# tsolomko/SWCompression

Measured on AMD Instinct MI355X. Metric: decompressed GiB/s, higher is better.
Workload: dtype u8; 1 GPU; 100000 x 64 KiB gzip members (BASELINE configs[1]; 4096 distinct, tiled at distinct addresses); codec=deflate, units_per_gpu=100000, unit_bytes=65536, compressed_bytes_per_gpu=2122936095, decompressed_bytes_per_gpu=6553600000, parallelism=1 x independent shards (weak scaling)

## Files before the change

swcompression_amd/csrc/inflate_sync.h:

```cpp
#ifndef SWC_INFLATE_SYNC_H
#define SWC_INFLATE_SYNC_H

#include "inflate_lane.h"
#include "simt.h"
#include "sync_round.h"

namespace swc {
namespace inflate {

#ifndef SWC_SYNC_LIT_BITS
#define SWC_SYNC_LIT_BITS 10
#endif
constexpr int kSyncLitBits = SWC_SYNC_LIT_BITS, kSyncDistBits = 8;
constexpr uint32_t kSyncChunk = SWC_SYNC_CHUNK;
constexpr uint32_t kSyncRound = 64u * kSyncChunk;
constexpr uint32_t kSyncStage = (kSyncRound + 32u + 15u) & ~15u;
constexpr uint32_t kPosFail = 0xFFFFFFFFu;
#ifndef SWC_SYNC_WALK_BACK
#define SWC_SYNC_WALK_BACK 128
#endif
#ifndef SWC_COPY_REC
#define SWC_COPY_REC 16
#define SWC_COPY_LIT 8
#endif
constexpr uint32_t kSyncWalkBack = SWC_SYNC_WALK_BACK;
static_assert(kSyncChunk % 4 == 0 && kSyncChunk >= 36, "sub-chunks are whole dwords");

#ifndef SWC_SYNC_NO_PAIRS
#define SWC_SYNC_NO_PAIRS 0
#endif
#ifndef SWC_SYNC_NO_FOLLOW
#define SWC_SYNC_NO_FOLLOW 0
#endif
#ifndef SWC_SYNC_FOLLOW_HELD
#define SWC_SYNC_FOLLOW_HELD 0
#endif
#define SWC_SYNC_FOLLOW (SWC_SYNC_NO_FOLLOW ? 0 : SWC_SYNC_FOLLOW_HELD ? 2 : 1)
constexpr uint32_t kEntLenBit = (uint32_t)kSyncLitBits + 2u;
constexpr uint32_t kEntNotLen = ((1u << (kSyncLitBits - kSyncDistBits)) - 1u) << (kSyncDistBits + 2), kEntLen = 1u << kEntLenBit, kEntLit = 1u << 13, kEntDist = 1u << 29, kEntStop = 1u << 30, kEntTog = 1u << 31;
static_assert(kSyncLitBits > kSyncDistBits && kEntLenBit <= 12u, "the entry keeps bits 10 .. 12 for the table switch");
constexpr uint32_t kEntBaseShift = 14, kEntPosMask = kEntTog | kEntStop | 31u;
constexpr uint32_t kLitMask4 = ((1u << kSyncLitBits) - 1u) << 2, kDistMask4 = ((1u << kSyncDistBits) - 1u) << 2;
static_assert(kEntLen == 4u << kSyncLitBits, "the length flag is the byte offset of the distance table");
static_assert(((((uint32_t)kSyncLitBits + 2u) << 10) & kEntLen) != 0u && (kEntLit & (kEntLen | kEntNotLen)) == 0u, "a link has the literal bit AND the length bit, a literal only the first (the follow-up literal tells them apart by that)");
static_assert((kLitMask4 & ~kEntNotLen) == kDistMask4, "the masks differ in the not-length bits");
constexpr uint32_t kInvLit = 2u | kEntNotLen | kEntStop, kInvDist = kInvLit | kEntTog;
constexpr uint32_t kEntShShift = 23, kEntPairBit = 28, kEntPair = SWC_SYNC_NO_PAIRS ? 0u : 1u << kEntPairBit, kEntPairLenShift = 16, kPairLenMax = 127;
SWC_HD uint32_t make_entry(uint32_t clen, uint32_t ext, uint32_t kind, uint32_t mant, uint32_t sh) {
    const uint32_t c = (clen + ext + 2u) | ((clen + 2u) << 5);
    const uint32_t v = SWC_SYNC_NO_PAIRS ? (mant << sh) << kEntBaseShift : (mant << kEntBaseShift) | (sh << kEntShShift);
    return kind == 1 ? c | kEntNotLen | kEntLit | v
         : kind == 2 ? c | kEntLen | kEntTog | v
         : kind == 3 ? c | kEntNotLen | kEntStop
                     : c | kEntNotLen | kEntDist | kEntTog | v;
}
SWC_HD uint32_t ent_bits(uint32_t e) { return (e & 31u) - 2u; }
SWC_HD uint32_t ent_code_bits(uint32_t e) { return ((e >> 5) & 31u) - 2u; }
SWC_HD bool ent_is_eob(uint32_t e) { return (e & kEntStop) != 0u && (e & 31u) > 2u; }
SWC_HD bool ent_is_link(uint32_t e) { return (e & kEntPosMask) == 0u; }
SWC_HD bool ent_is_pair(uint32_t e) { return (e & kEntPair) != 0u; }
SWC_HD uint32_t ent_pair_len(uint32_t e) { return bfe32(e, kEntPairLenShift, 7); }
SWC_HD uint32_t ent_base(uint32_t e) {
    if (SWC_SYNC_NO_PAIRS) return bfe32(e, kEntBaseShift, 15);
    return bfe32(e, kEntBaseShift, ent_is_pair(e) ? 2u : 9u) << bfe32(e, kEntShShift, 4);
}
SWC_HD uint32_t pair_entry(uint32_t e, uint32_t idx, const uint32_t* dlut) {
    if (SWC_SYNC_NO_PAIRS || ent_is_link(e) || (e & (kEntLen | kEntStop)) != kEntLen) return 0u;
    const uint32_t nl = ent_bits(e), cl = ent_code_bits(e);
    if (nl >= (uint32_t)kSyncLitBits) return 0u;
    const uint32_t r = (uint32_t)kSyncLitBits - nl;
    const uint32_t len = ent_base(e) + ((idx >> cl) & ((1u << (nl - cl)) - 1u));
    if (len > kPairLenMax) return 0u;
    const uint32_t de = dlut[(idx >> nl) & ((1u << kSyncDistBits) - 1u)];
    if (ent_is_link(de) || (de & (kEntDist | kEntStop)) != kEntDist) return 0u;
    const uint32_t d = ent_code_bits(de);
    if (d > r) return 0u;
    const uint32_t c2 = nl + d + 2u, n2 = c2 + (ent_bits(de) - d);
    return n2 | (c2 << 5) | kEntNotLen | kEntDist | kEntPair | (len << kEntPairLenShift) | (de & ((3u << kEntBaseShift) | (15u << kEntShShift)));
}

SWC_HD uint32_t entry_of_symbol(bool dist, uint32_t sym, uint32_t d) {
    if (!dist) {
        if (sym < 256) return make_entry(d, 0, 1, sym, 0);
        if (sym == 256) return make_entry(d, 0, 3, 0, 0);
        if (sym > 285) return kInvLit;
        const uint32_t s = sym - 257u;
        const uint32_t e = s < 8 || s == 28 ? 0u : (s >> 2) - 1u;
        const uint32_t base = s < 8 ? 3u + s : s == 28 ? 258u : 3u + ((4u + (s & 3u)) << e);
        return make_entry(d, e, 2, base, 0);
    }
    if (sym > 29) return kInvDist;
    const uint32_t e = sym < 4 ? 0u : (sym >> 1) - 1u;
    return make_entry(d, e, 0, sym < 4 ? sym : 2u + (sym & 1u), e);
}

constexpr int kAuxLim = 0, kAuxSlot = 16, kAuxStart = 32, kAuxCount = 48 , kAuxOver = 49, kAuxTable = 52;
constexpr int kAuxLit = 0, kAuxDist = kAuxTable, kAuxWords = 2 * kAuxTable;
constexpr uint32_t kSpillSyms = 512, kSpillSub = 1536, kSubLds = 184, kSubMax = (uint32_t)(lzr::kProvSpillBytes - kSpillSub) / 4u;
constexpr uint32_t kSymDist = 288;
static_assert(kAuxWords * 4 <= (int)kSpillSyms && kSpillSyms + 2 * (288 + 32) <= kSpillSub && kSubMax < 4096u, "spill layout");

struct SyncLds {
    alignas(16) uint8_t stage[kSyncStage];
    uint32_t lut[(1 << kSyncLitBits) + (1 << kSyncDistBits)];
    uint32_t sub[kSubLds];
};
#if SWC_SYNC_CHUNK == 68 && SWC_SYNC_LIT_BITS == 10
static_assert(sizeof(SyncLds) == 10240, "16 waves per CU: the wave's LDS must stay within 160 KB / 16");
#endif
constexpr uint32_t kHdrLens = 0;
constexpr uint32_t kHdrRun = 320;
constexpr uint32_t kHdrClLut = 512;
constexpr uint32_t kHdrSorted = 640;
constexpr uint32_t kHdrRank = 1280;
constexpr uint32_t kHdrIn = 1280;
constexpr uint32_t kHdrPt = 1280;
constexpr uint32_t kHdrTab = 3840;
static_assert(kHdrTab + 2 * 33 * 4 <= kSyncStage && kHdrPt + 2 * 1280 <= kHdrTab, "header scratch fits the stage");

enum { kSyncEob = 0, kSyncBail = 1, kSyncBailCap = 2 };
#if defined(SWC_HOST_EMULATION)
inline uint64_t g_sync_stats[8];
#define SWC_SYNC_STAT(i, n) (g_sync_stats[i] += (n))
inline uint64_t g_sync_iters = 0, g_sync_wave[4] = {0, 0, 0, 0}, g_sync_passmax = 0, g_sync_it0 = 0;
inline uint8_t g_sync_long[4096];
#define SWC_SYNC_ITER() (g_sync_iters++)
#define SWC_SYNC_LONG() (g_sync_long[(g_sync_iters - 1 - g_sync_it0) & 4095] = 1)
#define SWC_SYNC_LANE_BEGIN(first) if (first) { g_sync_passmax = 0; for (auto& h_ : g_sync_long) h_ = 0; } g_sync_it0 = g_sync_iters;
#define SWC_SYNC_LANE_END(last, k) { if (g_sync_iters - g_sync_it0 > g_sync_passmax) g_sync_passmax = g_sync_iters - g_sync_it0; if (last) { g_sync_wave[k] += g_sync_passmax; for (auto h_ : g_sync_long) g_sync_wave[3] += h_; } }
#else
#define SWC_SYNC_STAT(i, n) ((void)0)
#define SWC_SYNC_ITER() ((void)0)
#define SWC_SYNC_LONG() ((void)0)
#define SWC_SYNC_LANE_BEGIN(first)
#define SWC_SYNC_LANE_END(last, k)
#endif
enum { kFlagEob = 1u, kFlagFail = 2u, kFlagTrap = 4u, kFlagSlow = 8u };
#if defined(SWC_PROFILE) && defined(__HIP_DEVICE_COMPILE__)
struct SyncProf {
    uint64_t acc[16] = {0, 0, 0, 0, 0, 0, 0, 0, 0, 0, 0, 0, 0, 0, 0, 0};
    uint64_t tlast = 0;
};
#define SWC_SP(pp, k) { const uint64_t t_ = __builtin_readcyclecounter(); (pp).acc[k] += t_ - (pp).tlast; (pp).tlast = t_; }
#define SWC_SPC(pp, k, n) ((pp).acc[k] += (n))
#else
struct SyncProf {};
#define SWC_SP(pp, k)
#define SWC_SPC(pp, k, n)
#endif

struct SubTab {
    const SWC_AS_GLOBAL uint32_t* g;
};
struct Spill {
    SWC_AS_GLOBAL uint32_t* aux;
    SWC_AS_GLOBAL uint16_t* syms;
    SWC_AS_GLOBAL uint32_t* sub;
};

SWC_D uint32_t stage_bits(const SyncLds* sl, uint32_t p) {
    const uint32_t* w = (const uint32_t*)(sl->stage + ((p >> 3) & 0x1FFCu));
    return funnel32(w[1], w[0], p);
}
SWC_D uint32_t long_lookup(const SyncLds* sl, const SubTab st, uint32_t bits4, uint32_t link) {
    const uint32_t idx = bfe32(bits4, link >> 10, link >> 5);
    const uint32_t at = (link >> 18) + idx;
    return st.g ? st.g[at] : sl->sub[at < kSubLds ? at : 0u];
}
SWC_D uint32_t entry_at(const SyncLds* sl, const SubTab st, uint32_t pos, bool dist, uint32_t& bits4) {
    bits4 = stage_bits(sl, pos);
    uint32_t e = *(const uint32_t*)((const uint8_t*)sl->lut + ((bits4 & (dist ? kDistMask4 : kLitMask4)) | (dist ? kEntLen : 0u)));
    if (ent_is_link(e)) e = long_lookup(sl, st, bits4, e);
    return e;
}

template <bool LIT>
SWC_D int decode_sym_canon(BitReader& br, const Spill sp) {
    const SWC_AS_GLOBAL uint32_t* tb = sp.aux + (LIT ? kAuxLit : kAuxDist);
    const uint32_t c15 = brev32(br.peek32()) >> 17;
    uint32_t len = 16, idx = 0;
    if (tb[kAuxOver] == 0) {
        len = 1;
#pragma unroll 1
        for (int d = 1; d <= 15; d++) len += c15 >= tb[kAuxLim + d] ? 1u : 0u;
        if (len > 15) return -1;
        idx = (tb[kAuxSlot + len] + (c15 >> (15 - len))) & 0xFFFFu;
    } else {
#pragma unroll 1
        for (uint32_t d = 1; d <= 15; d++) {
            const uint32_t st = tb[kAuxStart + d], cnt = (tb[kAuxStart + d + 1] - st) & 0xFFFFu;
            const uint32_t fst = d == 1 ? 0u : tb[kAuxLim + d - 1] >> (15 - d);
            const uint32_t k0 = ((c15 >> (15 - d)) - fst) & ((1u << d) - 1u);
            if (k0 < cnt) {
                len = d;
                idx = st + k0 + (((cnt - 1u - k0) >> d) << d);
                break;
            }
        }
        if (len > 15) return -1;
    }
    if (len > br.bc) return -1;
    br.consume(len);
    if (idx >= (LIT ? 288u : 32u)) return -1;
    return (int)sp.syms[(LIT ? 0u : kSymDist) + idx];
}

SWC_D int careful_step(Lane& ln, const Spill sp) {
    BitReader& br = ln.br;
    br.refill();
    const int sym = decode_sym_canon<true>(br, sp);
    if (sym < 0) return SWC_E_DEFLATE_SYMBOL_NOT_FOUND;
    if (sym < 256) {
        ln.put_byte((uint8_t)sym);
        return SWC_OK;
    }
    if (sym == 256) return -1;
    if (sym > 285) return SWC_E_DEFLATE_WRONG_SYMBOL;
    const uint32_t s = (uint32_t)sym - 257u;
    uint32_t length;
    if (s < 8) {
        length = 3 + s;
    } else if (s == 28) {
        length = 258;
    } else {
        const uint32_t e = (s >> 2) - 1;
        if (br.bc < e) return SWC_E_DEFLATE_SYMBOL_NOT_FOUND;
        length = 3 + ((4 + (s & 3)) << e) + br.bits(e);
    }
    br.refill();
    const int dc = decode_sym_canon<false>(br, sp);
    if (dc < 0) return SWC_E_DEFLATE_SYMBOL_NOT_FOUND;
    if (dc > 29) return SWC_E_DEFLATE_WRONG_SYMBOL;
    uint32_t distance;
    if (dc < 4) {
        distance = 1 + (uint32_t)dc;
    } else {
        const uint32_t e = ((uint32_t)dc >> 1) - 1;
        if (br.bc < e) return SWC_E_DEFLATE_SYMBOL_NOT_FOUND;
        distance = 1 + ((2 + ((uint32_t)dc & 1)) << e) + br.bits(e);
    }
    if ((uint64_t)distance > ln.pos) {
        const uint32_t over = distance - (uint32_t)ln.pos;
        if (over > ln.back) return SWC_E_REF_TRAP;
        if (over > ln.reach) ln.reach = over;
    }
    ln.emit_match(length, distance);
    return SWC_OK;
}

SWC_D void table_from_counts(const uint32_t* cnt, SWC_AS_GLOBAL uint32_t* tb, uint32_t* first, uint32_t* start) {
    uint32_t v = 0, off = 0, over = 0;
    tb[kAuxLim] = 0; tb[kAuxSlot] = 0; tb[kAuxStart] = 0;
    first[0] = 0; start[0] = 0;
#pragma unroll 1
    for (int d = 1; d <= 15; d++) {
        const uint32_t c = cnt[d];
        tb[kAuxLim + d] = (v + c) << (15 - d);
        if (c != 0 && v + c > (1u << d)) over = 1;
        tb[kAuxSlot + d] = (off - v) & 0xFFFFu;
        tb[kAuxStart + d] = off;
        first[d] = v;
        start[d] = off;
        off += c;
        v = (v + c) << 1;
    }
    tb[kAuxCount] = off;
    tb[kAuxOver] = over;
    start[16] = off;
}

SWC_D bool sync_tables_from_lengths(SyncLds* sl, const Spill sp, int literals, int distances, SubTab& st, SyncProf& pf) {
    SWC_SP(pf, 0)
    using simt::PT;
    constexpr int N = kWave;
    const uint8_t* lens = sl->stage + kHdrLens;
    uint32_t* run = (uint32_t*)(sl->stage + kHdrRun);
    uint16_t* sorted = (uint16_t*)(sl->stage + kHdrSorted);
    uint16_t* rankb = (uint16_t*)(sl->stage + kHdrRank);
    uint16_t* pt = (uint16_t*)(sl->stage + kHdrPt);
    uint32_t* tab = (uint32_t*)(sl->stage + kHdrTab);
    const int total = literals + distances;
    st.g = nullptr;
    SIMT_BEGIN(t, N) if (t < 32) run[t] = 0; SIMT_END_WAVE
    PT<uint32_t, N> v, upd;
    PT<uint64_t, N> m;
    PT<bool, N> p;
#pragma unroll 1
    for (int g = 0; g * N < literals + N; g++) {
        const bool is_dist = g * N >= literals;
        const int s0 = is_dist ? literals : g * N, s_end = is_dist ? total : literals;
        SIMT_BEGIN(t, N) v[t] = s0 + t < s_end ? (uint32_t)lens[s0 + t] : 0u; m[t] = ~0ull; SIMT_END
#pragma unroll
        for (int k = 0; k < 4; k++) {
            SIMT_BEGIN(t, N) p[t] = ((v[t] >> k) & 1u) != 0u; SIMT_END
            const uint64_t b = simt::wave_ballot<N>(p);
            SIMT_BEGIN(t, N) m[t] &= p[t] ? b : ~b; SIMT_END
        }
        SIMT_BEGIN(t, N)
            upd[t] = 0;
            if (v[t] != 0u) {
                const uint32_t rank = (uint32_t)simt::popc64(m[t] & ((1ull << t) - 1ull)), cnt = (uint32_t)simt::popc64(m[t]);
                const uint32_t base = run[(is_dist ? 16u : 0u) + v[t]];
                rankb[s0 + t] = (uint16_t)(base + rank);
                if (rank == cnt - 1u) upd[t] = base + cnt;
            }
        SIMT_END_WAVE
        SIMT_BEGIN(t, N) if (upd[t] != 0u) run[(is_dist ? 16u : 0u) + v[t]] = upd[t]; SIMT_END_WAVE
    }
    SWC_SP(pf, 10)
    SIMT_BEGIN(t, N)
        if (t < 2) table_from_counts(run + 16 * t, sp.aux + (t ? kAuxDist : kAuxLit), tab + 33 * t, tab + 33 * t + 16);
    SIMT_END_WAVE
    SIMT_BEGIN(t, N)
        for (int s = t; s < total; s += N) {
            const uint32_t d = lens[s];
            if (d) {
                const bool dd = s >= literals;
                const uint32_t j = (dd ? kSymDist : 0u) + tab[(dd ? 33 : 0) + 16 + d] + rankb[s];
                const uint32_t sym = (uint32_t)(s - (dd ? literals : 0));
                if (j < kSymDist + 32u) { sorted[j] = (uint16_t)(sym | (d << 9)); sp.syms[j] = (uint16_t)sym; }
            }
        }
        for (int i = t; i < (1 << kSyncLitBits) + (1 << kSyncDistBits); i += N) sl->lut[i] = i < (1 << kSyncLitBits) ? kInvLit : kInvDist;
    SIMT_END_WAVE
    simt::vmem_fence();
    SWC_SP(pf, 11)
    if (sp.aux[kAuxLit + kAuxOver] != 0u || sp.aux[kAuxDist + kAuxOver] != 0u) return false;
    uint32_t used = 0, used_lit = 0;
    PT<uint32_t, N> sz, rv, ln2;
#pragma unroll 1
    for (int tbl = 0; tbl < 2; tbl++) {
        const uint32_t root = tbl ? (uint32_t)kSyncDistBits : (uint32_t)kSyncLitBits, rmask = (1u << root) - 1u;
        const uint32_t* first = tab + 33 * tbl;
        const uint32_t* start = first + 16;
        const uint32_t n_sym = start[16] < (tbl ? 32u : 288u) ? start[16] : (tbl ? 32u : 288u);
        const uint16_t* srt = sorted + (tbl ? kSymDist : 0u);
        uint32_t* lut = sl->lut + (tbl ? (1 << kSyncLitBits) : 0);
        uint16_t* ptt = pt + (tbl ? (1 << kSyncLitBits) : 0);
#pragma unroll 1
        for (uint32_t j0 = 0; j0 < n_sym; j0 += (uint32_t)N) {
            SIMT_BEGIN(t, N)
                const uint32_t j = j0 + (uint32_t)t;
                sz[t] = 0; ln2[t] = 0; rv[t] = 0;
                if (j < n_sym) {
                    const uint32_t w = srt[j], sym = w & 511u, d = w >> 9;
                    const uint32_t code = first[d] + (j - start[d]);
                    const uint32_t rev = brev32(code) >> (32u - d);
                    rv[t] = rev; ln2[t] = d;
                    if (d <= root) {
                        const uint32_t entry = entry_of_symbol(tbl != 0, sym, d);
                        for (uint32_t q = rev; q <= rmask; q += 1u << d) lut[q] = entry;
                    } else {
                        bool last = j + 1u == n_sym;
                        if (!last) {
                            const uint32_t w2 = srt[j + 1u], d2 = w2 >> 9;
                            const uint32_t rev2 = brev32(first[d2] + (j + 1u - start[d2])) >> (32u - d2);
                            last = (rev2 & rmask) != (rev & rmask);
                        }
                        if (last) sz[t] = 1u << (d - root);
                    }
                }
            SIMT_END
            PT<uint32_t, N> x = sz;
            simt::wave_scan_incl<N>(x);
            SIMT_BEGIN(t, N)
                if (sz[t] != 0u) {
                    const uint32_t at = used + x[t] - sz[t], k = ln2[t] - root, pre = rv[t] & rmask;
                    if (at + sz[t] <= kSubMax) {
                        ptt[pre] = (uint16_t)(at | (k << 12));
                        lut[pre] = (k << 5) | ((root + 2u) << 10) | (at << 18);
                    }
                }
            SIMT_END
            used += simt::wave_read<N>(x, N - 1);
        }
        if (tbl == 0) used_lit = used;
    }
    SWC_SP(pf, 12)
    if (used > kSubMax) return false;
    SWC_AS_GLOBAL uint32_t* subg = used > kSubLds ? sp.sub : nullptr;
    st.g = subg;
    simt::wave_fence();
#if !SWC_SYNC_NO_PAIRS
    SIMT_BEGIN(t, N)
        for (int i = t; i < (1 << kSyncLitBits); i += N) {
            const uint32_t pe2 = pair_entry(sl->lut[i], (uint32_t)i, sl->lut + (1 << kSyncLitBits));
            if (pe2 != 0u) sl->lut[i] = pe2;
        }
    SIMT_END
#endif
    SIMT_BEGIN(t, N)
        for (uint32_t i = (uint32_t)t; i < used; i += (uint32_t)N) {
            const uint32_t inv = i < used_lit ? kInvLit : kInvDist;
            if (subg) subg[i] = inv; else sl->sub[i] = inv;
        }
    SIMT_END_WAVE
    if (subg) simt::vmem_fence();
#pragma unroll 1
    for (int tbl = 0; tbl < 2; tbl++) {
        const uint32_t root = tbl ? (uint32_t)kSyncDistBits : (uint32_t)kSyncLitBits, rmask = (1u << root) - 1u;
        const uint32_t* first = tab + 33 * tbl;
        const uint32_t* start = first + 16;
        const uint32_t n_sym = start[16] < (tbl ? 32u : 288u) ? start[16] : (tbl ? 32u : 288u);
        if (start[root + 1] >= n_sym) continue;
        const uint16_t* srt = sorted + (tbl ? kSymDist : 0u);
        const uint16_t* ptt = pt + (tbl ? (1 << kSyncLitBits) : 0);
        SIMT_BEGIN(t, N)
            for (uint32_t j = start[root + 1] + (uint32_t)t; j < n_sym; j += (uint32_t)N) {
                const uint32_t w = srt[j], sym = w & 511u, d = w >> 9;
                const uint32_t rev = brev32(first[d] + (j - start[d])) >> (32u - d);
                const uint32_t entry = entry_of_symbol(tbl != 0, sym, d);
                const uint32_t pw = ptt[rev & rmask], at = pw & 0xFFFu, k = pw >> 12;
                for (uint32_t q = rev >> root; q < (1u << k); q += 1u << (d - root)) {
                    if (subg) subg[at + q] = entry; else sl->sub[at + q] = entry;
                }
            }
        SIMT_END
    }
    simt::wave_fence();
    if (subg) simt::vmem_fence();
    SWC_SP(pf, 13)
    return true;
}

SWC_D uint32_t walk_chunk(const SyncLds* sl, const SubTab st, uint32_t start, uint32_t chunk_end, uint32_t in_bits) {
    if (chunk_end > in_bits) chunk_end = in_bits;
    if (start >= in_bits) return kPosFail;
    uint32_t pos = start, tm = kLitMask4, tb = 0, e = 0;
    uint32_t c_notlen = kEntNotLen, c_dmask = kDistMask4;
    SWC_OPAQUE(c_notlen); SWC_OPAQUE(c_dmask);
    if (start < chunk_end) do {
        SWC_SYNC_STAT(4, 1);
        SWC_SYNC_ITER();
        const uint32_t bits4 = stage_bits(sl, pos);
        e = *(const uint32_t*)((const uint8_t*)sl->lut + and_or(bits4, tm, tb));
        uint32_t mm = e & kEntPosMask;
        if (mm == 0u) { SWC_SYNC_STAT(7, 1); SWC_SYNC_LONG(); e = long_lookup(sl, st, bits4, e); mm = e & kEntPosMask; }
        pos = pos + mm + 0xFFFFFFFEu;
        tm = and_or(e, c_notlen, c_dmask);
        tb = e & kEntLen;
    } while ((int32_t)pos < (int32_t)chunk_end);
    const uint32_t endb = pos & 0x3FFFFFFFu;
    const bool fail = ((pos & kEntStop) != 0u && !ent_is_eob(e)) || endb > in_bits;
    return fail ? kPosFail : endb;
}

struct ProvOut {
    uint32_t end, nlit, nrec, nout, flags, tail;
    int32_t need;
};
using sround::kProvRow;

template <bool NEED>
SWC_D void decode_chunk_prov(const SyncLds* sl, const SubTab st, uint32_t start, uint32_t chunk_end, uint32_t in_bits, gptr prov,
                             uint32_t lane, uint32_t run0, ProvOut& r) {
    const uint32_t rbase = 4u * lane;
#if !SWC_SYNC_FOLLOW
    const uint32_t lbase = (uint32_t)lzr::kProvRecBytes + 4u * lane;
#endif
    uint32_t pos = start, tm = kLitMask4, tb = 0, e = 0;
#if SWC_SYNC_FOLLOW
    const uint32_t lbase4 = (uint32_t)lzr::kProvRecBytes - kProvRow + 4u * lane;
    uint32_t plen = 0, run = run0, nl4 = 4, nout = 0, lb = 0;
#else
    uint32_t plen = 0, run = run0, nl3 = 3, nout = 0, lb = 0;
#endif
    uint32_t roff = rbase + kProvRow;
    int32_t need = -0x40000000;
    uint32_t c_notlen = kEntNotLen, c_dmask = kDistMask4;
    int32_t c_m256 = -256;
    SWC_OPAQUE(c_notlen); SWC_OPAQUE(c_dmask); SWC_OPAQUE(c_m256);
#if !SWC_SYNC_NO_PAIRS
    int32_t c_m4 = -4;
    SWC_OPAQUE(c_m4);
#endif
    if (chunk_end > in_bits) chunk_end = in_bits;
    const bool dead = start >= in_bits;
    uint32_t w0 = 0, w1 = 0;
    if (!dead && start < chunk_end) { const uint32_t* w = (const uint32_t*)(sl->stage + ((pos >> 3) & 0x1FFCu)); w0 = w[0]; w1 = w[1]; }
    if (!dead && start < chunk_end) do {
        SWC_SYNC_STAT(5, 1);
        SWC_SYNC_ITER();
        const uint32_t bits4 = funnel32(w1, w0, pos);
        e = *(const uint32_t*)((const uint8_t*)sl->lut + and_or(bits4, tm, tb));
        uint32_t mm = e & kEntPosMask;
        if (mm == 0u) { SWC_SYNC_STAT(7, 1); SWC_SYNC_LONG(); e = long_lookup(sl, st, bits4, e); mm = e & kEntPosMask; }
#if SWC_SYNC_FOLLOW == 2
        const uint32_t wbase = pos & ~31u;
#endif
        pos = pos + mm + 0xFFFFFFFEu;
#if SWC_SYNC_FOLLOW == 2
        const uint32_t fb4 = (uint32_t)((((uint64_t)w1 << 32) | w0) >> ((pos - wbase) & 63u));
        const uint32_t fend = wbase + (65u - kEntLenBit) < chunk_end ? wbase + (65u - kEntLenBit) : chunk_end;
#else
        { const uint32_t* w = (const uint32_t*)(sl->stage + ((pos >> 3) & 0x1FFCu)); w0 = w[0]; w1 = w[1]; }
#endif
        tm = and_or(e, c_notlen, c_dmask);
        tb = e & kEntLen;
#if SWC_SYNC_FOLLOW
#if SWC_SYNC_FOLLOW != 2
        const uint32_t fb4 = funnel32(w1, w0, pos);
        const uint32_t fend = chunk_end;
#endif
        const uint32_t f = *(const uint32_t*)((const uint8_t*)sl->lut + (fb4 & kLitMask4));
        const uint32_t fm = ((uint32_t)(pos < fend) & (uint32_t)((f & (kEntLit | kEntLen)) == kEntLit)) != 0u ? f : 2u;
        pos = pos + (fm & 31u) + 0xFFFFFFFEu;
        { const uint32_t* w = (const uint32_t*)(sl->stage + ((pos >> 3) & 0x1FFCu)); w0 = w[0]; w1 = w[1]; }
#endif
#if SWC_SYNC_NO_PAIRS
        const uint32_t val = (bfe32(bits4, 0, e) >> ((e >> 5) & 31u)) + bfe32(e, kEntBaseShift, 15);
        const uint32_t mlen = plen;
#else
        const uint32_t lp = bfe32(e, kEntPairLenShift, 7) & sbfe1(e, kEntPairBit);
        const uint32_t val = lshl_add_v(mad24(lp, c_m4, bfe32(e, kEntBaseShift, 9)), bfe32(e, kEntShShift, 4), bfe32(bits4, 0, e) >> ((e >> 5) & 31u));
        const uint32_t mlen = plen + lp;
#endif
        const uint32_t lit1 = bfe32(e, 13, 1);
        lb = alignbyte32(val, lb, lit1);
        const uint32_t dm = sbfe1(e, 29);
#if SWC_SYNC_FOLLOW
        const uint32_t lit2 = bfe32(fm, 13, 1), byte2 = fm >> kEntBaseShift, nl4_0 = nl4, litn = lit1 + lit2;
        nl4 += litn;
        if ((nl4 ^ nl4_0) > 3u) store_u32(prov + lshl_add<6>(nl4 & ~3u, lbase4), alignbyte32(byte2, lb, clear_if(nl4, lit2)));
        lb = alignbyte32(byte2, lb, lit2);
#else
        nl3 += lit1;
        const uint32_t litn = lit1;
        if (((nl3 & 3u) | (lit1 << 2)) == 7u) store_u32(prov + lshl_add<6>(nl3 & ~3u, lbase), lb);
#endif
        if (dm != 0u) store_u32(prov + roff, lshl_add<7>(mlen, lshl_add<16>(val, run)));
        roff = mad24(dm, c_m256, roff);
        if (NEED) {
            const int32_t nd = (int32_t)val - (int32_t)nout;
            need = (int32_t)bfi32(dm, (uint32_t)(nd > need ? nd : need), (uint32_t)need);
        }
        nout += litn + mlen;
#if SWC_SYNC_FOLLOW
        run = bfi32(dm, lit2, run + litn);
#else
        run = clear_if(dm, run + lit1);
#endif
        plen = val & sbfe1(e, kEntLenBit);
    } while ((int32_t)pos < (int32_t)chunk_end);
#if SWC_SYNC_FOLLOW
    const uint32_t nlit = nl4 - 4u;
    if (nlit & 3u) store_u32(prov + lshl_add<6>((nl4 & ~3u) + 4u, lbase4), lb);
#else
    const uint32_t nlit = nl3 - 3u;
    if (nlit & 3u) store_u32(prov + lshl_add<6>(nl3 & ~3u, lbase), lb);
#endif
    const uint32_t endb = pos & 0x3FFFFFFFu;
    uint32_t flags = 0;
    if (dead) flags = kFlagFail;
    else if (pos & kEntStop) flags = ent_is_eob(e) ? kFlagEob : kFlagFail;
    uint32_t tail = 0;
    if (run > 0) {
        if (flags & kFlagEob) tail = run;
        else { store_u32(prov + roff, lzr::make_lits(run)); roff += kProvRow; }
    }
    if (endb > in_bits) flags |= kFlagFail;
    if (nlit + run0 > lzr::kLitRunMax) flags |= kFlagSlow;
    r.end = (flags & kFlagFail) ? kPosFail : endb;
    r.nlit = nlit; r.nrec = (roff - rbase) / kProvRow - 1u; r.nout = nout; r.flags = flags; r.tail = tail; r.need = need;
}

SWC_D void copy_prov(gcptr plit, gcptr prec, uint32_t nlit, uint32_t nrec, gptr ldst, SWC_AS_GLOBAL uint32_t* rdst) {
    sround::copy_prov<SWC_COPY_REC, SWC_COPY_LIT, true>(plit, prec, nlit, nrec, ldst, rdst);
}

struct ChunkOut {
    uint32_t end;
    uint32_t nlit, nrec, nout;
    uint32_t flags;
    uint32_t over;
};
template <int MODE, bool BIG, bool CHK>
SWC_D void decode_chunk(const SyncLds* sl, const SubTab st, uint32_t start, uint32_t chunk_end, uint32_t in_bits, gptr lit_dst,
                        SWC_AS_GLOBAL uint32_t* rec_dst, uint64_t out_pos0, ChunkOut& r, uint32_t back = 0) {
    uint32_t pos = start;
    bool dist_next = false;
    uint32_t plen = 0, run = 0, nlit = 0, nrec = 0, nout = 0, flags = 0, over = 0;
    uint32_t lb = 0, lbn = 0;
    const uint32_t own = out_pos0 > 0x40000000ull ? 0x40000000u : (uint32_t)out_pos0;
    const uint32_t room = own + back;
    for (;;) {
        if (!dist_next && pos >= chunk_end) break;
        SWC_SYNC_STAT(4 + MODE, 1);
        SWC_SYNC_ITER();
        uint32_t bits4;
        const uint32_t e = entry_at(sl, st, pos, dist_next, bits4);
        const uint32_t n = ent_bits(e);
        if ((e & kEntStop) || (CHK && pos + n > in_bits)) {
            if (!ent_is_eob(e) || (CHK && pos + n > in_bits)) flags |= kFlagFail;
            else { pos += n; flags |= kFlagEob; }
            break;
        }
        const bool was_dist = dist_next || ent_is_pair(e);
        if (ent_is_pair(e)) plen = ent_pair_len(e);
        const uint32_t is_lit = (e >> 13) & 1u;
        const uint32_t val = (bfe32(bits4, 0, e) >> ((e >> 5) & 31u)) + ent_base(e) + (was_dist ? 1u : 0u);
        if (MODE != 0 && was_dist && val > own + nout) {
            if (val > room + nout) { flags |= kFlagTrap; break; }
            if (val - (own + nout) > over) over = val - (own + nout);
        }
        const bool big = BIG && was_dist && run > lzr::kLitRunMax;
        if (MODE == 1) {
            if (is_lit) {
                lb = funnel32(val, lb, 8);
                if (++lbn == 4) { store_u32(lit_dst, lb); lit_dst += 4; lbn = 0; }
            }
            if (was_dist) {
                if (big) *rec_dst++ = lzr::make_lits(run);
                *rec_dst++ = lzr::make_match(big ? 0u : run, plen, val);
            }
        }
        nlit += is_lit;
        nout += is_lit + (was_dist ? plen : 0u);
        nrec += was_dist ? (big ? 2u : 1u) : 0u;
        run = was_dist ? 0u : run + is_lit;
        plen = (e & kEntLen) ? val : plen;
        dist_next = (e & kEntLen) != 0u;
        pos += n;
    }
    if (run > 0) {
        nrec++;
        if (MODE == 1) *rec_dst++ = lzr::make_lits(run);
    }
    if (MODE == 1) {
        for (uint32_t i = 0; i < lbn; i++) lit_dst[i] = (uint8_t)(lb >> (8 * (4u - lbn + i)));
    }
    r.end = (flags & kFlagFail) ? kPosFail : pos;
    r.nlit = nlit; r.nrec = nrec; r.nout = nout;
    r.flags = flags;
    r.over = over;
}

template <int N>
SWC_D void stage_round(SyncLds* sl, gcptr in, uint32_t in_len, uint32_t B, uint32_t first_start, simt::PT<uint32_t, N>& start) {
    using simt::PT;
    constexpr uint32_t kParts = (kSyncStage + 16u * N - 1u) / (16u * N);
    PT<uint64_t, N> sa[kParts], sb[kParts];
    PT<uint32_t, N> sp[kParts];
    SIMT_BEGIN(t, N)
#pragma unroll
        for (uint32_t k = 0; k < kParts; k++) {
            const uint32_t o = 16u * (uint32_t)t + k * 16u * N;
            uint64_t a = 0, b = 0;
            uint32_t prev = 0;
            const uint64_t at = (uint64_t)B + o;
            if (o < kSyncStage) {
                if (at + 16 <= in_len) {
                    a = load_u64(in + at); b = load_u64(in + at + 8);
                    if (o != 0) prev = load_u32(in + at - 4);
                } else {
                    for (uint32_t q = 0; q < 8; q++) if (at + q < in_len) a |= (uint64_t)in[at + q] << (8 * q);
                    for (uint32_t q = 0; q < 8; q++) if (at + 8 + q < in_len) b |= (uint64_t)in[at + 8 + q] << (8 * q);
                    if (o != 0) for (uint32_t q = 0; q < 4; q++) if (at - 4 + q < in_len) prev |= (uint32_t)in[at - 4 + q] << (8 * q);
                }
            }
            sa[k][t] = a; sb[k][t] = b; sp[k][t] = prev;
        }
    SIMT_END
    SIMT_BEGIN(t, N)
#pragma unroll
        for (uint32_t k = 0; k < kParts; k++) {
            const uint32_t o = 16u * (uint32_t)t + k * 16u * N;
            if (o < kSyncStage) {
                uint32_t* st32 = (uint32_t*)(sl->stage + o);
                const uint64_t a = sa[k][t], b = sb[k][t];
                const uint32_t w0 = (uint32_t)a, w1 = (uint32_t)(a >> 32), w2 = (uint32_t)b, w3 = (uint32_t)(b >> 32);
                st32[0] = funnel32(w0, sp[k][t], 30); st32[1] = funnel32(w1, w0, 30); st32[2] = funnel32(w2, w1, 30); st32[3] = funnel32(w3, w2, 30);
            }
        }
        start[t] = t == 0 ? first_start : (uint32_t)t * kSyncChunk * 8u - kSyncWalkBack;
    SIMT_END_WAVE
}
SWC_D bool redo_lane(int t, uint32_t& start, uint32_t pe, bool have) {
    const bool todo = t == 0 ? !have : pe != kPosFail && (start != pe || !have);
    if (todo && t != 0) start = pe;
    return todo;
}
SWC_D bool stopped_in_front(uint32_t start, uint32_t chunk_end) { return start + kSyncChunk * 8u < chunk_end; }
template <class R>
SWC_D void nothing_taken(R& r) {
    r = R{};
    r.end = kPosFail; r.flags = kFlagFail;
}
template <int N>
SWC_D bool prov_turn(int t, const SyncLds* sl, const SubTab st, uint32_t in_bits, gptr prov, bool need, uint32_t run0,
                     simt::PT<uint32_t, N>& start, const simt::PT<uint32_t, N>& pe, simt::PT<bool, N>& have, simt::PT<uint32_t, N>& endp,
                     simt::PT<uint32_t, N>& c_lit, simt::PT<uint32_t, N>& c_rec, simt::PT<uint32_t, N>& c_out, simt::PT<uint32_t, N>& flg,
                     simt::PT<uint32_t, N>& c_tail, simt::PT<uint32_t, N>& c_need) {
    if (!redo_lane(t, start[t], pe[t], have[t])) return false;
    ProvOut r;
    const uint32_t ce = ((uint32_t)t + 1u) * kSyncChunk * 8u;
    if (stopped_in_front(start[t], ce)) nothing_taken(r);
    else if (need) decode_chunk_prov<true>(sl, st, start[t], ce, in_bits, prov, (uint32_t)t, run0, r);
    else decode_chunk_prov<false>(sl, st, start[t], ce, in_bits, prov, (uint32_t)t, run0, r);
    endp[t] = r.end; c_lit[t] = r.nlit; c_rec[t] = r.nrec; c_out[t] = r.nout; flg[t] = r.flags;
    c_tail[t] = r.tail; c_need[t] = (uint32_t)r.need;
    have[t] = true;
    return true;
}

#ifndef SWC_TEAM_WAVES
#define SWC_TEAM_WAVES 6
#endif
#if defined(SWC_HOST_EMULATION)
inline uint64_t g_team_adopted = 0;
#define SWC_TEAM_STAT() (g_team_adopted++)
#else
#define SWC_TEAM_STAT() ((void)0)
#endif
constexpr int kTeamWaves = SWC_TEAM_WAVES;
constexpr uint32_t kTeamStride = 63u * kSyncChunk;
constexpr size_t kTeamProvBytes = lzr::kProvRecBytes + lzr::kProvLitBytes;
struct TeamRound {
    uint32_t c_lit[kWave], c_rec[kWave];
    uint32_t nv, eob, ok;
    uint32_t start1;
    uint32_t end_last, tail_last;
    uint32_t tot_lit, tot_rec, tot_out;
    uint32_t mneed;
// ... 330 lines not shown
                        else decode_chunk<0, true, false>(sl, st, start[t], ce, in_bits, nullptr, nullptr, 0, r);
                    }
                    endp[t] = r.end; c_lit[t] = r.nlit; c_rec[t] = r.nrec; c_out[t] = r.nout; flg[t] = r.flags;
                    have[t] = true;
                }
                SWC_SYNC_LANE_END(t_i_ == N - 1, 1)
            SIMT_END
            SWC_SP(pf, 3)
        }
        if (bail) { SWC_SYNC_STAT(1, 1); break; }
        SWC_SYNC_STAT(0, 1);
        const sround::Totals tot = sround::lane_offsets<N>(0u, nv, c_lit, c_rec, c_out, x_lit, x_rec, x_out);
        SWC_SP(pf, 4)
        const bool beyond = pos >= ln.cap;
        if (!beyond && pos + tot.out > ln.cap) { result = kSyncBailCap; break; }
        if (!beyond && (uint64_t)nrec + tot.rec > ln.max_rec) break;
        SIMT_BEGIN(t, N)
            SWC_SYNC_LANE_BEGIN(t_i_ == 0)
            if ((uint32_t)t < nv) {
                ChunkOut r;
                const uint32_t ce = ((uint32_t)t + 1u) * kSyncChunk * 8u;
                const uint64_t p0 = pos + (x_out[t] - c_out[t]);
                const bool bigs = c_lit[t] > lzr::kLitRunMax;
                if (beyond) decode_chunk<2, false, true>(sl, st, start[t], ce, in_bits, nullptr, nullptr, p0, r, back);
                else if (bigs || chk) decode_chunk<1, true, true>(sl, st, start[t], ce, in_bits, ln.lits + nlit + (x_lit[t] - c_lit[t]), ln.recs + nrec + (x_rec[t] - c_rec[t]), p0, r, back);
                else decode_chunk<1, false, false>(sl, st, start[t], ce, in_bits, ln.lits + nlit + (x_lit[t] - c_lit[t]), ln.recs + nrec + (x_rec[t] - c_rec[t]), p0, r, back);
                flg[t] = r.flags;
                c_need[t] = r.over;
            }
            SWC_SYNC_LANE_END(t_i_ == N - 1, 2)
        SIMT_END
        SWC_SP(pf, 5)
        SIMT_BEGIN(t, N) pb[t] = (uint32_t)t < nv && (flg[t] & kFlagTrap) != 0; SIMT_END
        if (simt::wave_ballot<N>(pb)) break;
        if (back != 0u && pos < 32768u) {
            SIMT_BEGIN(t, N) c_need[t] = (uint32_t)t < nv ? c_need[t] : 0u; SIMT_END
            simt::wave_scan_max_incl<N>(c_need);
            const uint32_t rr = simt::wave_read<N>(c_need, N - 1);
            if (rr > ln.reach) ln.reach = rr;
        }
        pos += tot.out;
        if (!beyond) { nlit += tot.lit; nrec += tot.rec; }
        P = 8ull * B + simt::wave_read<N>(endp, (int)nv - 1);
        ln.last_end = pos < ln.cap ? pos : (ln.last_end > ln.cap ? ln.last_end : ln.cap);
        if (eob) { result = kSyncEob; break; }
    }
    ln.pos = pos;
    ln.nlit = nlit;
    ln.nrec = nrec;
    ln.br.seek(P);
    return result;
}

SWC_D int build_dynamic_par(Lane& ln, SyncLds* sl, const Spill sp, SubTab& st, bool& fast, SyncProf& pf) {
    using simt::PT;
    constexpr int N = kWave;
    BitReader& br = ln.br;
    br.refill();
    if (br.bc < 14) return SWC_E_DEFLATE_SYMBOL_NOT_FOUND;
    const int literals = (int)br.bits(5) + 257;
    if (literals > 286) return SWC_E_DEFLATE_WRONG_SYMBOL;
    const int distances = (int)br.bits(5) + 1;
    const int ncl = (int)br.bits(4) + 4;
    br.refill();
    const uint64_t total_left = (uint64_t)br.len * 8 - br.consumed_bits();
    if (total_left < (uint64_t)(3 * ncl)) return SWC_E_DEFLATE_SYMBOL_NOT_FOUND;
    const uint8_t order[19] = {16, 17, 18, 0, 8, 7, 9, 6, 10, 5, 11, 4, 12, 3, 13, 2, 14, 1, 15};
    uint64_t clens = 0;
    for (int i = 0; i < ncl; i++) {
        br.refill();
        clens |= (uint64_t)br.bits(3) << (3 * order[i]);
    }
    Lane::ClTable cl;
    {
        uint64_t cnt8 = 0, runp = 0;
        for (int s = 0; s < 19; s++) {
            const uint32_t len = (uint32_t)(clens >> (3 * s)) & 7u;
            if (len) cnt8 += 1ull << (8 * len);
        }
        uint32_t v = 0, off = 0;
        cl.slot[0] = 0;
#pragma unroll
        for (int d = 1; d <= 7; d++) {
            const uint32_t c = (uint32_t)(cnt8 >> (8 * d)) & 255u;
            cl.slot[d] = ((v & 0x7FFFu) << 9) | off;
            runp |= (uint64_t)off << (8 * d);
            off += c;
            v = (v + c) << 1;
        }
        cl.slot[8] = off;
        cl.sym_lo = cl.sym_hi = 0;
        for (int s = 0; s < 19; s++) {
            const uint32_t len = (uint32_t)(clens >> (3 * s)) & 7u;
            if (len) {
                const uint32_t p = (uint32_t)(runp >> (8 * len)) & 255u;
                runp += 1ull << (8 * len);
                if (p < 12) cl.sym_lo |= (uint64_t)s << (5 * p);
                else cl.sym_hi |= (uint64_t)s << (5 * (p - 12));
            }
        }
    }
    SWC_SP(pf, 14)
    uint8_t* lens = sl->stage + kHdrLens;
    uint8_t* cl_lut = sl->stage + kHdrClLut;
    uint32_t* hin = (uint32_t*)(sl->stage + kHdrIn);
    const int total = literals + distances;
    const uint64_t end_bits = (uint64_t)br.len * 8;
    uint64_t W = simt::uniform(br.consumed_bits());
    gcptr in = br.in;
    const uint32_t in_len = br.len;
    SIMT_BEGIN(t, N)
        for (int i = t; i < 80; i += N) ((uint32_t*)lens)[i] = 0;
        for (int x = t; x < 128; x += N) {
            uint32_t len;
            const int idx = Lane::cl_lookup(cl, brev32((uint32_t)x) >> 17, len);
            const uint32_t sym = idx < 0 ? 0u : (uint32_t)((idx < 12 ? cl.sym_lo >> (5 * idx) : cl.sym_hi >> (5 * (idx - 12))) & 31u);
            cl_lut[x] = idx < 0 ? (uint8_t)0xFF : (uint8_t)(len | (sym << 3));
        }
    SIMT_END_WAVE
    SWC_SP(pf, 15)
    int n = 0;
    uint32_t prev = 0;
    uint64_t HB = ~0ull;
    PT<uint32_t, N> nxt, mlo, mhi, jmp, gl, gh, gj, src, symv, repv, errv, cbx, bef, key, kex;
    PT<bool, N> pb, actv;
    while (n < total) {
        if (HB == ~0ull || W + 64 + 32 > 8 * (HB + 1024)) {
            HB = (W >> 3) & ~3ull;
            SIMT_BEGIN(t, N)
                uint64_t a = 0, b = 0;
                const uint64_t at = HB + 16u * (uint32_t)t;
                if (at + 16 <= in_len) { a = load_u64(in + at); b = load_u64(in + at + 8); }
                else {
                    for (uint32_t k = 0; k < 8; k++) if (at + k < in_len) a |= (uint64_t)in[at + k] << (8 * k);
                    for (uint32_t k = 0; k < 8; k++) if (at + 8 + k < in_len) b |= (uint64_t)in[at + 8 + k] << (8 * k);
                }
                uint32_t* h4 = hin + 4 * t;
                h4[0] = (uint32_t)a; h4[1] = (uint32_t)(a >> 32); h4[2] = (uint32_t)b; h4[3] = (uint32_t)(b >> 32);
                if (t < 4) hin[256 + t] = 0;
            SIMT_END_WAVE
        }
        const uint32_t rel0 = (uint32_t)(W - 8 * HB);
        const uint64_t left64 = end_bits - W;
        const uint32_t left = left64 > 0xFFFFu ? 0xFFFFu : (uint32_t)left64;
        SIMT_BEGIN(t, N)
            const uint32_t rel = rel0 + (uint32_t)t;
            const uint32_t* w = hin + (rel >> 5);
            const uint32_t bits = funnel32(w[1], w[0], rel);
            const uint32_t e = cl_lut[bits & 127u];
            const uint32_t len = e & 7u, sym = e == 0xFFu ? 0u : e >> 3;
            const uint32_t xb = sym == 16u ? 2u : sym == 17u ? 3u : sym == 18u ? 7u : 0u;
            const uint32_t xv = bfe32(bits, len, xb);
            const uint32_t avail = left > (uint32_t)t ? left - (uint32_t)t : 0u;
            symv[t] = sym;
            repv[t] = sym < 16u ? 1u : sym == 18u ? 11u + xv : 3u + xv;
            errv[t] = e == 0xFFu || len > avail ? 1u : len + xb > avail ? 2u : 0u;
            nxt[t] = (uint32_t)t + (e == 0xFFu ? 1u : len + xb);
            jmp[t] = nxt[t];
            mlo[t] = t < 32 ? 1u << t : 0u;
            mhi[t] = t < 32 ? 0u : 1u << (t - 32);
        SIMT_END
#pragma unroll 1
        for (int k = 0; k < 6; k++) {
            if (simt::uniform(simt::wave_read<N>(jmp, 0)) >= 64u) break;
            SIMT_BEGIN(t, N) src[t] = jmp[t] < 64u ? jmp[t] : (uint32_t)t; SIMT_END
            simt::wave_gather<N>(gl, mlo, src);
            simt::wave_gather<N>(gh, mhi, src);
            simt::wave_gather<N>(gj, jmp, src);
            SIMT_BEGIN(t, N) if (jmp[t] < 64u) { mlo[t] |= gl[t]; mhi[t] |= gh[t]; jmp[t] = gj[t]; } SIMT_END
        }
        const uint64_t V = ((uint64_t)simt::uniform(simt::wave_read<N>(mhi, 0)) << 32) | simt::uniform(simt::wave_read<N>(mlo, 0));
        SIMT_BEGIN(t, N) cbx[t] = (V >> t) & 1ull ? repv[t] : 0u; SIMT_END
        simt::wave_scan_incl<N>(cbx);
        SIMT_BEGIN(t, N)
            const bool vis = ((V >> t) & 1ull) != 0ull;
            const uint32_t rep = repv[t], before = (uint32_t)n + cbx[t] - (vis ? rep : 0u), sym = symv[t];
            const bool act = vis && before < (uint32_t)total;
            uint32_t err = 0;
            if (act) {
                if (errv[t] == 1u) err = (uint32_t)SWC_E_DEFLATE_SYMBOL_NOT_FOUND;
                else if (sym == 16u && before == 0u) err = (uint32_t)SWC_E_DEFLATE_WRONG_SYMBOL;
                else if (sym >= 16u && errv[t] == 2u) err = (uint32_t)SWC_E_DEFLATE_SYMBOL_NOT_FOUND;
                else if (sym == 16u && before + rep > (uint32_t)total) err = (uint32_t)SWC_E_DEFLATE_WRONG_SYMBOL;
            }
            errv[t] = err;
            pb[t] = err != 0u;
            actv[t] = act;
            bef[t] = before;
            key[t] = act && sym != 16u ? (((uint32_t)t + 1u) << 8) | (sym < 16u ? sym : 0u) : 0u;
        SIMT_END
        {
            const uint64_t m_err = simt::wave_ballot<N>(pb);
            if (m_err) return (int)simt::wave_read<N>(errv, simt::ctz64(m_err));
        }
        kex = key;
        simt::wave_scan_max_incl<N>(kex);
        const uint32_t klast = simt::uniform(simt::wave_read<N>(kex, N - 1));
        simt::wave_shift_up<N>(key, kex, 0u);
        SIMT_BEGIN(t, N)
            if (actv[t]) {
                const uint32_t sym = symv[t];
                const uint32_t val = sym < 16u ? sym : sym == 16u ? (key[t] ? key[t] & 255u : prev) : 0u;
                if (val != 0u) for (uint32_t k = 0; k < repv[t]; k++) lens[bef[t] + k] = (uint8_t)val;
            }
        SIMT_END
        const uint64_t m_act = simt::wave_ballot<N>(actv);
        const int last = 63 - simt::clz64(m_act);
        n = (int)(simt::uniform(simt::wave_read<N>(bef, last)) + simt::uniform(simt::wave_read<N>(repv, last)));
        W += simt::uniform(simt::wave_read<N>(nxt, last));
        if (klast) prev = klast & 255u;
    }
    if (n != total) return SWC_E_DEFLATE_WRONG_SYMBOL;
    simt::wave_fence();
    br.seek(W);
    SWC_SP(pf, 0)
    fast = sync_tables_from_lengths(sl, sp, literals, distances, st, pf);
    return SWC_OK;
}

SWC_D void build_static_par(SyncLds* sl, const Spill sp, SubTab& st, bool& fast, SyncProf& pf) {
    constexpr int N = kWave;
    uint8_t* lens = sl->stage + kHdrLens;
    SIMT_BEGIN(t, N)
        for (int s = t; s < 320; s += N) lens[s] = (uint8_t)(s < 144 ? 8 : s < 256 ? 9 : s < 280 ? 7 : s < 288 ? 8 : 5);
    SIMT_END_WAVE
    fast = sync_tables_from_lengths(sl, sp, 288, 32, st, pf);
}

template <bool TEAM = false>
SWC_D void inflate_sync_job(Job& job, SyncLds* sl, uint8_t* ws, size_t ws_bytes, int lane, int lanes, uint64_t* prof = nullptr, Team* tm = nullptr) {
    Lane ln;
    SyncProf pf;
#if defined(SWC_PROFILE) && defined(__HIP_DEVICE_COMPILE__)
    pf.tlast = __builtin_readcyclecounter();
#endif
    ln.wlane = lane;
    ln.wlanes = lanes;
    ln.l = LaneLds{nullptr, 1};
    ln.out = (gptr)job.out;
    ln.cap = job.out_cap;
    ln.pos = 0;
    ln.nrec = 0;
    ln.nlit = 0;
    ln.last_end = 0;
    const size_t lo = ws ? lzr::lit_offset(ws_bytes, job.out_cap) : 0;
    ln.recs = (SWC_AS_GLOBAL uint32_t*)(ws + sizeof(lzr::StreamHeader));
    size_t rec_end = lo;
    ln.prov = nullptr;
    if (lo >= sizeof(lzr::StreamHeader) + 256 + lzr::kProvBytes) {
        rec_end = (lo - lzr::kProvBytes) & ~(size_t)15;
        ln.prov = (gptr)(ws + rec_end);
    }
    ln.max_rec = rec_end > sizeof(lzr::StreamHeader) ? (uint32_t)((rec_end - sizeof(lzr::StreamHeader)) / 4) : 0u;
    ln.lits = (gptr)(ws + lo);
    Spill sp{nullptr, nullptr, nullptr};
    if (ln.prov) {
        gptr s0 = ln.prov + lzr::kProvRecBytes + lzr::kProvLitBytes;
        sp.aux = (SWC_AS_GLOBAL uint32_t*)s0;
        sp.syms = (SWC_AS_GLOBAL uint16_t*)(s0 + kSpillSyms);
        sp.sub = (SWC_AS_GLOBAL uint32_t*)(s0 + kSpillSub);
    }
    int st = SWC_OK;
    const bool open = (job.aux & kDeflateOpen) != 0;
    bool ended_open = false;
    const bool linked = (job.aux & kDeflateLinked) != 0;
    ln.back = linked ? 32768u : 0u;
    if (linked && (job.aux & kDeflateJoined) == 0) {
        st = SWC_E_INVALID_ARGUMENT;
        ln.br.init((gcptr)job.in, 0, 0);
    } else if (lo == 0 || ln.prov == nullptr) {
        st = SWC_E_NEED_WORKSPACE;
        ln.br.init((gcptr)job.in, 0, 0);
    } else if (job.in_len > 0xFFFFFFF0ull) {
        st = SWC_E_INVALID_ARGUMENT;
        ln.br.init((gcptr)job.in, 0, 0);
    } else {
        ln.br.init((gcptr)job.in, (uint32_t)job.in_len, 0);
        if ((uint64_t)ln.br.len * 8 < 10) st = SWC_E_DEFLATE_WRONG_BLOCK_TYPE;
        while (st == SWC_OK) {
            ln.br.refill();
            if (open && ln.br.bc == 0) { ended_open = true; break; }
            if (ln.br.bc < 3) { st = SWC_E_REF_TRAP; break; }
            const uint32_t is_last = ln.br.bits(1);
            const uint32_t type = ln.br.bits(2);
            if (type == 0) {
                st = ln.run_stored();
            } else if (type == 1 || type == 2) {
                SWC_SP(pf, 6)
                bool fast = false;
                SubTab stb{nullptr};
                if (type == 1) build_static_par(sl, sp, stb, fast, pf);
                else st = build_dynamic_par(ln, sl, sp, stb, fast, pf);
                SWC_SP(pf, 1)
                if constexpr (TEAM) if (tm != nullptr) tm->gen++;
                if (st == SWC_OK) {
                    for (;;) {
                        if (fast) {
                            const int r = sync_block<TEAM>(ln, sl, stb, pf, tm);
                            if (r == kSyncEob) break;
                            if (r == kSyncBail) fast = false;
                        }
                        const uint64_t until = fast && ln.pos < ln.cap ? ln.cap : ~0ull;
                        int s2 = SWC_OK;
                        do { s2 = careful_step(ln, sp); } while (s2 == SWC_OK && ln.pos < until && until != ~0ull);
                        if (s2 == -1) break;
                        if (s2) { st = s2; break; }
                    }
                }
            } else {
                st = SWC_E_DEFLATE_WRONG_BLOCK_TYPE;
            }
            if (st != SWC_OK || is_last) break;
        }
        ln.flush_tail();
    }
    if constexpr (TEAM) if (tm != nullptr && tm->sh != nullptr) team_dismiss(*tm);
    if (ln.nrec > ln.max_rec) {
        st = SWC_E_NEED_WORKSPACE;
        ln.nrec = ln.max_rec;
    }
    if (st == SWC_OK && ln.pos > ln.cap) st = SWC_E_CAPACITY;
    if (ws && ws_bytes >= sizeof(lzr::StreamHeader) && (lane == 0)) {
        SWC_AS_GLOBAL lzr::StreamHeader* h = (SWC_AS_GLOBAL lzr::StreamHeader*)ws;
        h->nrec = ln.nrec;
        h->pad0 = ln.reach;
        h->nlit = ln.nlit;
    }
#if defined(SWC_PROFILE) && defined(__HIP_DEVICE_COMPILE__)
    SWC_SP(pf, 6)
    if (prof && lane == 0) for (int k = 0; k < 16; k++) prof[k] = pf.acc[k];
#else
    (void)prof; (void)pf;
#endif
    const uint64_t bits = ln.br.consumed_bits();
    const uint64_t consumed = (bits + 7) >> 3;
    job.in_consumed = consumed > job.in_len ? job.in_len : consumed;
    job.out_len = ln.pos;
    job.status = st;
    if (!ended_open) job.aux &= ~kDeflateOpen;
}

}
}
#endif
```

Before: 472.6 GiB/s.

## Parallelize Huffman count tables with wave scans and skip redundant LUT invalidation

Replaces the serial two-lane table_from_counts loop with wave-wide inclusive scans over the 32 length counts, computing limit, start and first codes per lane and detecting oversubscription with a ballot. The invalid-entry prefill of the lit/dist LUTs now runs only when the code is incomplete or over-subscribed, and overflowing subtable prefixes are invalidated directly. The pair-entry loop visits rows in bit-reversed order. The global memory fence moves from the table build to the end of the build and before the careful-step path. This is meant to cut per-block dynamic header cost, with some risk to correctness around fence placement and incomplete codes.

```diff
diff --git a/swcompression_amd/csrc/inflate_sync.h b/swcompression_amd/csrc/inflate_sync.h
--- a/swcompression_amd/csrc/inflate_sync.h
+++ b/swcompression_amd/csrc/inflate_sync.h
@@ -246,27 +246,6 @@
     }
     ln.emit_match(length, distance);
     return SWC_OK;
-}
-
-SWC_D void table_from_counts(const uint32_t* cnt, SWC_AS_GLOBAL uint32_t* tb, uint32_t* first, uint32_t* start) {
-    uint32_t v = 0, off = 0, over = 0;
-    tb[kAuxLim] = 0; tb[kAuxSlot] = 0; tb[kAuxStart] = 0;
-    first[0] = 0; start[0] = 0;
-#pragma unroll 1
-    for (int d = 1; d <= 15; d++) {
-        const uint32_t c = cnt[d];
-        tb[kAuxLim + d] = (v + c) << (15 - d);
-        if (c != 0 && v + c > (1u << d)) over = 1;
-        tb[kAuxSlot + d] = (off - v) & 0xFFFFu;
-        tb[kAuxStart + d] = off;
-        first[d] = v;
-        start[d] = off;
-        off += c;
-        v = (v + c) << 1;
-    }
-    tb[kAuxCount] = off;
-    tb[kAuxOver] = over;
-    start[16] = off;
 }
 
 SWC_D bool sync_tables_from_lengths(SyncLds* sl, const Spill sp, int literals, int distances, SubTab& st, SyncProf& pf) {
@@ -308,9 +287,40 @@
         SIMT_BEGIN(t, N) if (upd[t] != 0u) run[(is_dist ? 16u : 0u) + v[t]] = upd[t]; SIMT_END_WAVE
     }
     SWC_SP(pf, 10)
+    PT<uint32_t, N> cc, lim, off;
     SIMT_BEGIN(t, N)
-        if (t < 2) table_from_counts(run + 16 * t, sp.aux + (t ? kAuxDist : kAuxLit), tab + 33 * t, tab + 33 * t + 16);
+        cc[t] = t < 32 ? run[t] : 0u;
+        lim[t] = cc[t] << (15 - (t & 15));
+        off[t] = cc[t];
+    SIMT_END
+    simt::wave_scan_incl<N>(lim);
+    simt::wave_scan_incl<N>(off);
+    const uint32_t lim_lit = simt::uniform(simt::wave_read<N>(lim, 15)), off_lit = simt::uniform(simt::wave_read<N>(off, 15));
+    const uint32_t lim_dist = simt::uniform(simt::wave_read<N>(lim, 31)) - lim_lit;
+    SIMT_BEGIN(t, N)
+        if (t >= 16) { lim[t] -= lim_lit; off[t] -= off_lit; }
+        p[t] = t < 32 && cc[t] != 0u && lim[t] > (1u << 15);
+    SIMT_END
+    const uint32_t over_mask = (uint32_t)simt::wave_ballot<N>(p);
+    const bool over = over_mask != 0u;
+    SIMT_BEGIN(t, N)
+        if (t < 32) {
+            const uint32_t d = (uint32_t)t & 15u, a = (uint32_t)t >> 4;
+            const uint32_t first = (lim[t] - (cc[t] << (15u - d))) >> (15u - d), start = off[t] - cc[t];
+            SWC_AS_GLOBAL uint32_t* tb = sp.aux + (a ? kAuxDist : kAuxLit);
+            tb[kAuxLim + d] = lim[t];
+            tb[kAuxSlot + d] = (start - first) & 0xFFFFu;
+            tb[kAuxStart + d] = start;
+            tab[33u * a + d] = first;
+            tab[33u * a + 16u + d] = start;
+            if (d == 15u) {
+                tb[kAuxCount] = off[t];
+                tb[kAuxOver] = ((over_mask >> (16u * a)) & 0xFFFFu) != 0u ? 1u : 0u;
+                tab[33u * a + 32u] = off[t];
+            }
+        }
     SIMT_END_WAVE
+    const bool fill_lit = over || lim_lit != (1u << 15), fill_dist = over || lim_dist != (1u << 15);
     SIMT_BEGIN(t, N)
         for (int s = t; s < total; s += N) {
             const uint32_t d = lens[s];
@@ -321,11 +331,11 @@
                 if (j < kSymDist + 32u) { sorted[j] = (uint16_t)(sym | (d << 9)); sp.syms[j] = (uint16_t)sym; }
             }
         }
-        for (int i = t; i < (1 << kSyncLitBits) + (1 << kSyncDistBits); i += N) sl->lut[i] = i < (1 << kSyncLitBits) ? kInvLit : kInvDist;
+        if (fill_lit) for (int i = t; i < (1 << kSyncLitBits); i += N) sl->lut[i] = kInvLit;
+        if (fill_dist) for (int i = t; i < (1 << kSyncDistBits); i += N) sl->lut[(1 << kSyncLitBits) + i] = kInvDist;
     SIMT_END_WAVE
-    simt::vmem_fence();
     SWC_SP(pf, 11)
-    if (sp.aux[kAuxLit + kAuxOver] != 0u || sp.aux[kAuxDist + kAuxOver] != 0u) return false;
+    if (over) return false;
     uint32_t used = 0, used_lit = 0;
     PT<uint32_t, N> sz, rv, ln2;
 #pragma unroll 1
@@ -369,6 +379,8 @@
                     if (at + sz[t] <= kSubMax) {
                         ptt[pre] = (uint16_t)(at | (k << 12));
                         lut[pre] = (k << 5) | ((root + 2u) << 10) | (at << 18);
+                    } else {
+                        lut[pre] = tbl ? kInvDist : kInvLit;
                     }
                 }
             SIMT_END
@@ -383,14 +395,17 @@
     simt::wave_fence();
 #if !SWC_SYNC_NO_PAIRS
     SIMT_BEGIN(t, N)
-        for (int i = t; i < (1 << kSyncLitBits); i += N) {
-            const uint32_t pe2 = pair_entry(sl->lut[i], (uint32_t)i, sl->lut + (1 << kSyncLitBits));
+        for (int r = t; r < (1 << kSyncLitBits); r += N) {
+            const uint32_t i = brev32((uint32_t)r) >> (32u - (uint32_t)kSyncLitBits);
+            const uint32_t pe2 = pair_entry(sl->lut[i], i, sl->lut + (1 << kSyncLitBits));
             if (pe2 != 0u) sl->lut[i] = pe2;
         }
     SIMT_END
 #endif
     SIMT_BEGIN(t, N)
-        for (uint32_t i = (uint32_t)t; i < used; i += (uint32_t)N) {
+        uint32_t i0 = (uint32_t)t;
+        SWC_OPAQUE(i0);
+        for (uint32_t i = i0; i < used; i += (uint32_t)N) {
             const uint32_t inv = i < used_lit ? kInvLit : kInvDist;
             if (subg) subg[i] = inv; else sl->sub[i] = inv;
         }
@@ -418,7 +433,7 @@
         SIMT_END
     }
     simt::wave_fence();
-    if (subg) simt::vmem_fence();
+    simt::vmem_fence();
     SWC_SP(pf, 13)
     return true;
 }
@@ -1355,6 +1370,7 @@
                         }
                         const uint64_t until = fast && ln.pos < ln.cap ? ln.cap : ~0ull;
                         int s2 = SWC_OK;
+                        simt::vmem_fence();
                         do { s2 = careful_step(ln, sp); } while (s2 == SWC_OK && ln.pos < until && until != ~0ull);
                         if (s2 == -1) break;
                         if (s2) { st = s2; break; }
```

Result: no change. 473.4 GiB/s, median of 4 (+0.2%).
